# AmandineBtto/NeRAF

Hardware: AMD Instinct MI355X
Metric: field-samples/sec (rays + RIR STFT bins) (higher is better)
Workload: dtype f16; 1 GPU; RAF FurnishedRoom joint training step (BASELINE configs[2]): 4096 rays + 2048 RIR slices x 513 bins per GPU; radiance + grid refresh + ResNet3D + NAcF + STFT loss, backward, GradScaler + fused Adam...; rays_per_gpu=4096, slices_per_gpu=2048, global_rays=4096, global_slices=2048, parallelism=dp1, distinct_resident_batches=16, deterministic=True

## Files before the change

include/neraf_hip.h:

```cpp
#ifndef NERAF_HIP_H
#define NERAF_HIP_H

#include <stddef.h>
#include <stdint.h>

#ifdef __cplusplus
extern "C" {
#endif

typedef struct neraf_ctx neraf_ctx;
typedef void* neraf_stream_t;

enum {
  NERAF_OK = 0,
  NERAF_EINVAL = -1,
  NERAF_EHIP = -2,
  NERAF_ENOGPU = -3,
  NERAF_ESTATE = -4
};

#define NERAF_ABI_VERSION 1

int neraf_abi_version(void);
int neraf_ctx_create(neraf_ctx** out, int device);
void neraf_ctx_destroy(neraf_ctx* ctx);
const char* neraf_last_error(neraf_ctx* ctx);

int neraf_graph_stats(neraf_ctx* ctx, int* captures, int* launches);
int neraf_prof_enable(neraf_ctx* ctx, int on);
int neraf_prof_summary(neraf_ctx* ctx, int kernel_id, double* total_ms, int* launches, double* work);
int neraf_prof_summary_ex(neraf_ctx* ctx, int kernel_id, double* total_ms, int* launches, double* work, double* exec_work);
int neraf_prof_event_overhead(neraf_ctx* ctx, void* scratch_word, neraf_stream_t stream, double* ms);
const char* neraf_prof_kernel_name(int kernel_id);

int neraf_gemm_f16(neraf_ctx* ctx, const void* A, int lda, const void* B, int ldb, int M, int N, int K,
                   int Mpad, int Npad, float alpha, const float* bias, int act,
                   void* C16, int ldc16, void* C16T, int ldc16t, float* C32, int ldc32,
                   neraf_stream_t stream);

int neraf_gemm_f16_grouped(neraf_ctx* ctx, int ngroups, const void* const* A, const void* const* B, const int* M, const int* N,
                           float* const* C32, const int* ldc32, int lda, int ldb, int K, float alpha, const float* alpha_dev,
                           int c32_beta, void* splitk_ws, size_t splitk_bytes, neraf_stream_t stream);

int neraf_gemm_bf16(neraf_ctx* ctx, const void* A, int lda, const void* B, int ldb, int M, int N, int K,
                    int Mpad, int Npad, float alpha, const float* bias, int act,
                    void* C16, int ldc16, void* C16T, int ldc16t, float* C32, int ldc32,
                    neraf_stream_t stream);
int neraf_gemm_bf16_tn(neraf_ctx* ctx, const void* A, const void* B, int M, int N, int K, float* C32, void* splitk_ws,
                       size_t splitk_bytes, neraf_stream_t stream);

typedef struct neraf_nacf_desc {
  int n_feat;
  int n_query;
  int W;
  int C;
  int F;
  int dense_l0;
} neraf_nacf_desc;

size_t neraf_nacf_packed_bytes(const neraf_nacf_desc* d);
size_t neraf_nacf_workspace_bytes(const neraf_nacf_desc* d, int B, int training);

int neraf_nacf_pack_weights(neraf_ctx* ctx, const neraf_nacf_desc* d, const float* const* weights,
                            void* packed, neraf_stream_t stream);

int neraf_nacf_encode_queries(neraf_ctx* ctx, const neraf_nacf_desc* d, const int64_t* time_query,
                              const double* mic_pose, const double* source_pose, const double* rot,
                              const float* aabb_host, int max_len, int B, void* workspace, int training,
                              neraf_stream_t stream);
int neraf_nacf_encode_queries_ex(neraf_ctx* ctx, const neraf_nacf_desc* d, const int64_t* time_query,
                                 const double* mic_pose, const double* source_pose, const double* rot, int pose_rows,
                                 const float* aabb_host, int max_len, int B, void* workspace, int training,
                                 neraf_stream_t stream);

int neraf_nacf_fwd(neraf_ctx* ctx, const neraf_nacf_desc* d, const void* packed, const float* const* weights,
                   const float* feat, int B, float* out, void* workspace, int training, neraf_stream_t stream);

int neraf_nacf_fwd_dense(neraf_ctx* ctx, const neraf_nacf_desc* d, const void* packed, const float* h, int B,
                         float* out, void* workspace, int training, neraf_stream_t stream);

int neraf_nacf_bwd(neraf_ctx* ctx, const neraf_nacf_desc* d, const void* packed, const float* const* weights,
                   const float* feat, int B, const float* out, const float* dout, float* const* grads,
                   float* dfeat, void* workspace, neraf_stream_t stream);

int neraf_nacf_bwd_dense(neraf_ctx* ctx, const neraf_nacf_desc* d, const void* packed, int B, const float* out,
                         const float* dout, float* const* grads, float* dh, void* workspace,
                         neraf_stream_t stream);

#define NERAF_STFT_SUMS_FLOATS (4 + 4 * 256)
int neraf_stft_loss_fwd(neraf_ctx* ctx, const float* pred, const float* gt, size_t n, int loss_type,
                        float* sums, float* losses, neraf_stream_t stream);
int neraf_stft_loss_sums(neraf_ctx* ctx, const float* pred, const float* gt, size_t n, int loss_type,
                         float* sums, neraf_stream_t stream);
int neraf_stft_loss_finalize(neraf_ctx* ctx, const float* sums, size_t n_total, const float* weights, float* losses,
                             neraf_stream_t stream);
// ... 200 lines not shown
```

neraf_amd/_lib.py:

```python
from __future__ import annotations

import ctypes as C
import os
from typing import Dict, Optional

_HERE = os.path.dirname(os.path.abspath(__file__))
LIB_PATH = os.environ.get("NERAF_HIP_LIB") or os.path.join(_HERE, "libneraf_hip.so")

_lib: Optional[C.CDLL] = None
_ctxs: Dict[int, C.c_void_p] = {}

c_fpp = C.POINTER(C.c_void_p)


class GridDesc(C.Structure):
    _fields_ = [("n_levels", C.c_int), ("base_res", C.c_int), ("max_res", C.c_int), ("log2_hashmap_size", C.c_int),
                ("n_features", C.c_int)]


class ResnetDesc(C.Structure):
    _fields_ = [("grid_size", C.c_int), ("in_channels", C.c_int), ("n_features", C.c_int)]


class NacfDesc(C.Structure):
    _fields_ = [("n_feat", C.c_int), ("n_query", C.c_int), ("W", C.c_int), ("C", C.c_int), ("F", C.c_int),
                ("dense_l0", C.c_int)]


SIGNATURES = {
    "neraf_abi_version": (C.c_int, []),
    "neraf_ctx_create": (C.c_int, [C.POINTER(C.c_void_p), C.c_int]),
    "neraf_ctx_destroy": (None, [C.c_void_p]),
    "neraf_last_error": (C.c_char_p, [C.c_void_p]),
    "neraf_gemm_f16": (C.c_int, [C.c_void_p, C.c_void_p, C.c_int, C.c_void_p, C.c_int, C.c_int, C.c_int, C.c_int,
                                 C.c_int, C.c_int, C.c_float, C.c_void_p, C.c_int, C.c_void_p, C.c_int, C.c_void_p,
                                 C.c_int, C.c_void_p, C.c_int, C.c_void_p]),
    "neraf_gemm_f16_grouped": (C.c_int, [C.c_void_p, C.c_int, c_fpp, c_fpp, C.POINTER(C.c_int), C.POINTER(C.c_int), c_fpp,
                                         C.POINTER(C.c_int), C.c_int, C.c_int, C.c_int, C.c_float, C.c_void_p, C.c_int, C.c_void_p, C.c_size_t,
                                         C.c_void_p]),
    "neraf_gemm_bf16": (C.c_int, [C.c_void_p, C.c_void_p, C.c_int, C.c_void_p, C.c_int, C.c_int, C.c_int, C.c_int,
                                  C.c_int, C.c_int, C.c_float, C.c_void_p, C.c_int, C.c_void_p, C.c_int, C.c_void_p,
                                  C.c_int, C.c_void_p, C.c_int, C.c_void_p]),
    "neraf_gemm_bf16_tn": (C.c_int, [C.c_void_p, C.c_void_p, C.c_void_p, C.c_int, C.c_int, C.c_int, C.c_void_p, C.c_void_p, C.c_size_t,
                                     C.c_void_p]),
    "neraf_fused_adam_chunk": (C.c_int, []),
    "neraf_grads_nonfinite": (C.c_int, [C.c_void_p, C.c_void_p, C.c_void_p, C.c_void_p, C.c_void_p, C.c_int, C.c_void_p, C.c_void_p, C.c_int,
                                        C.c_int, C.c_void_p]),
    "neraf_fused_adam": (C.c_int, [C.c_void_p, C.c_void_p, C.c_void_p, C.c_void_p, C.c_void_p, C.c_int, C.c_void_p, C.c_int, C.c_int,
                                   C.c_double, C.c_double, C.c_double, C.c_void_p, C.c_void_p, C.c_void_p, C.c_void_p]),
    "neraf_fused_adam_dual": (C.c_int, [C.c_void_p, C.c_void_p, C.c_void_p, C.c_void_p, C.c_void_p, C.c_int, C.c_void_p, C.c_int, C.c_int,
                                        C.c_double, C.c_double, C.c_double, C.c_void_p, C.c_void_p, C.c_void_p, C.c_void_p, C.c_void_p,
                                        C.c_void_p, C.c_void_p, C.c_int, C.c_void_p, C.c_int, C.c_void_p]),
    "neraf_nacf_packed_bytes": (C.c_size_t, [C.POINTER(NacfDesc)]),
    "neraf_nacf_workspace_bytes": (C.c_size_t, [C.POINTER(NacfDesc), C.c_int, C.c_int]),
    "neraf_nacf_pack_weights": (C.c_int, [C.c_void_p, C.POINTER(NacfDesc), c_fpp, C.c_void_p, C.c_void_p]),
    "neraf_nacf_encode_queries": (C.c_int, [C.c_void_p, C.POINTER(NacfDesc), C.c_void_p, C.c_void_p, C.c_void_p,
                                            C.c_void_p, C.POINTER(C.c_float), C.c_int, C.c_int, C.c_void_p, C.c_int,
                                            C.c_void_p]),
    "neraf_nacf_encode_queries_ex": (C.c_int, [C.c_void_p, C.POINTER(NacfDesc), C.c_void_p, C.c_void_p, C.c_void_p,
                                               C.c_void_p, C.c_int, C.POINTER(C.c_float), C.c_int, C.c_int, C.c_void_p, C.c_int,
                                               C.c_void_p]),
    "neraf_nacf_fwd": (C.c_int, [C.c_void_p, C.POINTER(NacfDesc), C.c_void_p, c_fpp, C.c_void_p, C.c_int, C.c_void_p,
                                 C.c_void_p, C.c_int, C.c_void_p]),
    "neraf_nacf_fwd_dense": (C.c_int, [C.c_void_p, C.POINTER(NacfDesc), C.c_void_p, C.c_void_p, C.c_int, C.c_void_p,
                                       C.c_void_p, C.c_int, C.c_void_p]),
    "neraf_nacf_bwd": (C.c_int, [C.c_void_p, C.POINTER(NacfDesc), C.c_void_p, c_fpp, C.c_void_p, C.c_int, C.c_void_p,
                                 C.c_void_p, c_fpp, C.c_void_p, C.c_void_p, C.c_void_p]),
    "neraf_nacf_bwd_dense": (C.c_int, [C.c_void_p, C.POINTER(NacfDesc), C.c_void_p, C.c_int, C.c_void_p, C.c_void_p,
                                       c_fpp, C.c_void_p, C.c_void_p, C.c_void_p]),
    "neraf_stft_loss_fwd": (C.c_int, [C.c_void_p, C.c_void_p, C.c_void_p, C.c_size_t, C.c_int, C.c_void_p, C.c_void_p,
                                      C.c_void_p]),
    "neraf_stft_loss_sums": (C.c_int, [C.c_void_p, C.c_void_p, C.c_void_p, C.c_size_t, C.c_int, C.c_void_p, C.c_void_p]),
    "neraf_stft_loss_finalize": (C.c_int, [C.c_void_p, C.c_void_p, C.c_size_t, C.c_void_p, C.c_void_p, C.c_void_p]),
    "neraf_stft_loss_bwd": (C.c_int, [C.c_void_p, C.c_void_p, C.c_void_p, C.c_size_t, C.c_size_t, C.c_int, C.c_void_p,
                                      C.c_void_p, C.c_void_p, C.c_void_p, C.c_float, C.c_void_p, C.c_void_p]),
    "neraf_prof_event_overhead": (C.c_int, [C.c_void_p, C.c_void_p, C.c_void_p, C.POINTER(C.c_double)]),
    "neraf_graph_stats": (C.c_int, [C.c_void_p, C.POINTER(C.c_int), C.POINTER(C.c_int)]),
    "neraf_prof_enable": (C.c_int, [C.c_void_p, C.c_int]),
    "neraf_prof_summary": (C.c_int, [C.c_void_p, C.c_int, C.POINTER(C.c_double), C.POINTER(C.c_int), C.POINTER(C.c_double)]),
    "neraf_prof_summary_ex": (C.c_int, [C.c_void_p, C.c_int, C.POINTER(C.c_double), C.POINTER(C.c_int), C.POINTER(C.c_double),
                                        C.POINTER(C.c_double)]),
    "neraf_prof_kernel_name": (C.c_char_p, [C.c_int]),
    "neraf_grid_layout": (C.c_int, [C.POINTER(GridDesc), C.POINTER(C.c_float), C.POINTER(C.c_int), C.POINTER(C.c_uint32),
                                    C.POINTER(C.c_uint32)]),
    "neraf_hash_encode": (C.c_int, [C.c_void_p, C.POINTER(GridDesc), C.c_void_p, C.c_void_p, C.c_longlong, C.c_void_p, C.c_void_p]),
    "neraf_sample_uniform": (C.c_int, [C.c_void_p, C.c_int, C.c_int, C.c_float, C.c_float, C.c_void_p, C.c_uint64, C.c_void_p,
                                       C.c_void_p, C.c_void_p]),
    "neraf_proposal_density": (C.c_int, [C.c_void_p, C.POINTER(GridDesc), C.c_void_p, C.c_void_p, C.c_void_p, C.c_void_p,
                                         C.c_void_p, C.c_int, C.c_int, C.c_float, C.c_int, C.c_void_p, C.c_void_p]),
    "neraf_proposal_density_ex": (C.c_int, [C.c_void_p, C.POINTER(GridDesc), C.c_void_p, C.c_void_p, C.c_void_p, C.c_void_p,
                                            C.c_void_p, C.c_int64, C.c_int, C.c_int, C.c_float, C.c_int, C.c_void_p, C.c_void_p]),
    "neraf_pdf_resample_ex": (C.c_int, [C.c_void_p, C.c_void_p, C.c_void_p, C.c_void_p, C.c_int64, C.c_int, C.c_int, C.c_float,
# ... 163 lines not shown
```

neraf_amd/csrc/common.h:

```cpp
#pragma once
#include <hip/hip_runtime.h>
#include <stdint.h>
#include <stdio.h>
#include <new>
#include <string>
#include <vector>

#include "../../include/neraf_hip.h"

typedef _Float16 half_t;
typedef _Float16 half8 __attribute__((ext_vector_type(8)));
typedef _Float16 half4 __attribute__((ext_vector_type(4)));
typedef _Float16 half2v __attribute__((ext_vector_type(2)));
typedef __bf16 bf16_t;
typedef __bf16 bf16x8 __attribute__((ext_vector_type(8)));
typedef __bf16 bf16x4 __attribute__((ext_vector_type(4)));
typedef float f32x4 __attribute__((ext_vector_type(4)));
typedef float f32x16 __attribute__((ext_vector_type(16)));

enum { PROF_GEMM128 = 0, PROF_GEMM64 = 1, PROF_PROP_DENSITY = 2, PROF_FIELD_QUERY = 3, PROF_CONV = 4, PROF_PROP_BWD = 5, PROF_FIELD_BWD = 6,
       PROF_FIELD_SCATTER = 7, PROF_GEMM_WIDE = 8, PROF_WGRAD = 9, PROF_GEMM64_BF16 = 10, PROF_GEMM12864 = 11,
       PROF_CONV64_BF16 = 12, PROF_CONV12864 = 13, PROF_CONV128 = 14, PROF_CONV_STEM = 15, PROF_NUM_KERNELS = 16 };

struct ProfRec { hipEvent_t a, b; int kid; double work; double exec; };
// ... 123 lines not shown
  if (!words) return;
  size_t blocks = (words + 256 - 1) / 256;
  if (blocks > 4096) blocks = 4096;
  hipLaunchKernelGGL(neraf_zero3_kernel, dim3((unsigned)blocks), dim3(256), 0, st, (unsigned*)p0, w0, (unsigned*)p1, w1, (unsigned*)p2, w2);
}

static inline bool neraf_deterministic() {
  static const bool d = [] { const char* e = getenv("NERAF_DETERMINISTIC"); return e && atoi(e) != 0; }();
  return d;
}

static inline int round_up(int x, int m) { return (x + m - 1) / m * m; }
static inline size_t round_up_sz(size_t x, size_t m) { return (x + m - 1) / m * m; }

enum { ACT_NONE = 0, ACT_LEAKY = 1, ACT_TANH10 = 2, ACT_RELU = 3 };

struct ConvGeom {
  int loader;
  int din, dout, stride, pad, ksize, cin;
  int tflip;
  int tstride;
  int tclass;
  const half_t* zero_page;
};

struct GemmParams {
  const half_t* A; int lda;
  const half_t* B; int ldb;
  int M, N, K;
  int Mpad, Npad;
  float alpha;
  const float* alpha_dev;
  const float* bias;
  int act;
  const half_t* lmask; int ldmask;
  float mask_slope;
  const half_t* add16; int ldadd;
  half_t* C16; int ldc16;
  half_t* C16T; int ldc16t;
  float* C32; int ldc32;
  int c32_beta;
  float* colsum;
  float* colsumsq;
  int stat_rep, stat_stride;
  int stat_det;
  const half_t* bnb_x; int ldbnb;
  const half_t* bnb_mask;
  const float* bnb_fin; int bnb_cpad;
  ConvGeom conv;
  float* splitk_ws; size_t splitk_ws_bytes;
  int tile_n;
  double alg_flops;
  int bf16;
  int ngroups;
  struct Group { const half_t* A; const half_t* B; float* C32; int M, N, ldc32; int tile_begin; } grp[6];
};
constexpr int kMaxGemmGroups = 6;

int launch_gemm_f16(neraf_ctx* ctx, const GemmParams& p, hipStream_t stream);

struct WgradItem {
  const void* dy;
  const void* x;
  float* out;
  int cout, cin, cin_real, ksize, stride, pad, din, dout;
  int K;
  int alpha_idx;
};
int launch_wgrad_grouped(neraf_ctx* ctx, const WgradItem* items, int n, const half_t* zero_page, float* slab_ws, size_t slab_bytes,
                         const float* alpha_dev, hipStream_t stream, bool bf16 = false);

constexpr int kAmaxRep = 32, kAmaxStride = 64;
```

neraf_amd/csrc/gemm_f16.hip:

```cpp
#include "common.h"
#include <stdlib.h>
#include <type_traits>

namespace {

constexpr int BK = 64;

__device__ __forceinline__ float act_apply(float v, int act) {
  if (act == ACT_LEAKY) return v > 0.f ? v : 0.1f * v;
  if (act == ACT_TANH10) return 10.f * tanhf(v);
  if (act == ACT_RELU) return v > 0.f ? v : 0.f;
  return v;
}

template <bool BF> struct ET;
template <> struct ET<false> {
  typedef _Float16 s; typedef half8 v8; typedef half4 v4;
  static __device__ __forceinline__ f32x4 mfma(v8 a, v8 b, f32x4 c) { return __builtin_amdgcn_mfma_f32_16x16x32_f16(a, b, c, 0, 0, 0); }
};
template <> struct ET<true> {
  typedef __bf16 s; typedef bf16x8 v8; typedef bf16x4 v4;
  static __device__ __forceinline__ f32x4 mfma(v8 a, v8 b, f32x4 c) { return __builtin_amdgcn_mfma_f32_16x16x32_bf16(a, b, c, 0, 0, 0); }
};

// ... 679 lines not shown
  __shared__ float tile2[32][33];
  if (p.bnb_x) {
#pragma unroll
    for (int r = 0; r < 4; ++r) tile2[row][c4 + r] = v[r] * (((float)xv[r] - mu[r]) * rsqrtf(var[r] + 1e-5f));
  }
  if (p.C16) {
    E4 h;
#pragma unroll
    for (int r = 0; r < 4; ++r) h[r] = (E)v[r];
    *reinterpret_cast<E4*>(reinterpret_cast<E*>(p.C16) + (size_t)m * p.ldc16 + n) = h;
  }
  if (C32 && m < M) {
    float* dst = C32 + (size_t)m * ldc32 + n;
    if (n + 3 < N && (reinterpret_cast<size_t>(dst) & 15) == 0) {
      f32x4 o = v;
      if (p.c32_beta) o += *reinterpret_cast<const f32x4*>(dst);
      *reinterpret_cast<f32x4*>(dst) = o;
    } else {
#pragma unroll
      for (int r = 0; r < 4; ++r) if (n + r < N) dst[r] = v[r] + (p.c32_beta ? dst[r] : 0.f);
    }
  }
  __syncthreads();
  const int tx = t & 31, ty = t >> 5;
  if (p.C16T) {
#pragma unroll
    for (int i = 0; i < 4; ++i) {
      const int nn = n0 + ty + i * 8, mm = m0 + tx;
      reinterpret_cast<E*>(p.C16T)[(size_t)nn * p.ldc16t + mm] = (E)tile[tx][ty + i * 8];
    }
  }
  if ((p.colsum || p.colsumsq) && ty < 2) {
    float cs = 0.f;
    if (ty == 0) {
#pragma unroll 8
      for (int i = 0; i < 32; ++i) cs += tile[i][tx];
    } else if (p.bnb_x) {
#pragma unroll 8
      for (int i = 0; i < 32; ++i) cs += tile2[i][tx];
    } else {
#pragma unroll 8
      for (int i = 0; i < 32; ++i) { const float x = tile[i][tx]; cs += x * x; }
    }
    float* dst = ty == 0 ? p.colsum : p.colsumsq;
    if (p.stat_det) {
      if (dst) dst[(size_t)blockIdx.y * p.stat_stride + n0 + tx] = cs;
    } else {
      const int rep = p.stat_rep > 1 ? (blockIdx.y & (p.stat_rep - 1)) * p.stat_stride : 0;
      if (dst) atomicAdd(dst + rep + n0 + tx, cs);
    }
  }
}

static void gemm_manifest(neraf_ctx* ctx, const GemmParams& p, int loader, int splits, int bm, int bn, double flops, bool wide = false) {
  double out_elems = (double)p.M * p.N;
  double rA = loader == 0 ? (double)p.M * p.K * 2.0 : (double)p.conv.din * p.conv.din * p.conv.din * p.conv.cin * 2.0;
  double rB = (double)p.N * p.K * 2.0;
  const int ng = p.ngroups > 1 ? p.ngroups : 1;
  if (ng > 1) {
    out_elems = rA = rB = 0.0;
    for (int g = 0; g < ng; ++g) { out_elems += (double)p.grp[g].M * p.grp[g].N; rA += (double)p.grp[g].M * p.K * 2.0; rB += (double)p.grp[g].N * p.K * 2.0; }
  }
  const double epi_r = out_elems * 2.0 * ((p.add16 ? 1 : 0) + (p.lmask ? 1 : 0) + (p.bnb_mask ? 1 : 0) + (p.bnb_x ? 1 : 0));
  const double epi_w = out_elems * (2.0 * ((p.C16 ? 1 : 0) + (p.C16T ? 1 : 0)) + (p.C32 ? 4.0 : 0.0));
  const double slabs = (double)splits * ng * p.Mpad * p.Npad * 4.0;
  char nm[96];
  if (ng > 1)
    snprintf(nm, sizeof(nm), "gemm_f16_nt_pipe_kernel<%d, %d | plain, %d groups, %.0f results K=%d%s", bm, bn, ng, out_elems, p.K, splits > 1 ? " splitK" : "");
  else
    snprintf(nm, sizeof(nm), "%s<%d, %d | %s M=%d N=%d K=%d%s", wide ? "gemm_f16_nt_wide_kernel" : "gemm_f16_nt_pipe_kernel", bm, bn,
             loader == 0 ? "plain" : (p.conv.tflip ? "dgrad" : "conv"), p.M, p.N, p.K, splits > 1 ? " splitK" : "");
  if (splits > 1) {
    neraf_node(ctx, nm, flops, rA + rB, slabs);
    neraf_node(ctx, "splitk_reduce_kernel | K-split slabs -> result", 0.0, slabs + epi_r, epi_w);
  } else {
    neraf_node(ctx, nm, flops, rA + rB + epi_r, epi_w);
  }
}

template <int BM, int BN, int NST, int LOADER, int KS, bool BF, bool TC = false, int NW = 4, bool GRP = false>
int launch_pipe(neraf_ctx* ctx, const GemmParams& p_in, int splits, hipStream_t stream) {
  using PT = PipeTile<BM, BN, NST>;
  GemmParams p = p_in;
  if ((p.ngroups > 1) != GRP) return neraf_fail(ctx, NERAF_EINVAL, "gemm: grouped launches take the grouped instantiation");
  int grp_tiles = 0;
  if (GRP) {
    for (int g = 0; g < p.ngroups; ++g) {
      p.grp[g].tile_begin = grp_tiles;
      grp_tiles += ((p.grp[g].M + BM - 1) / BM) * ((p.grp[g].N + BN - 1) / BN);
    }
  }
  static bool attr_set = false;
  if (!attr_set) {
    NERAF_HIP_CHECK(ctx, hipFuncSetAttribute(reinterpret_cast<const void*>(&gemm_f16_nt_pipe_kernel<BM, BN, NST, LOADER, KS, BF, TC, NW, GRP>),
                                             hipFuncAttributeMaxDynamicSharedMemorySize, PT::LDS_BYTES));
    attr_set = true;
  }
  const int ng = p.ngroups > 1 ? p.ngroups : 1;
  const int ntiles = GRP ? grp_tiles : (p.Mpad / BM) * (p.Npad / BN);
  double flops = 2.0 * p.M * p.N * p.K;
  if (ng > 1) { flops = 0.0; for (int g = 0; g < ng; ++g) flops += 2.0 * p.grp[g].M * p.grp[g].N * p.K; }
  const double exec_flops = (LOADER != 0 && p.conv.tstride > 1) ? (p.alg_flops > 0.0 ? p.alg_flops : flops) : flops;
  if (p.alg_flops > 0.0) flops = p.alg_flops;
  constexpr int kid = LOADER == 2 ? PROF_CONV_STEM
                      : LOADER == 1 ? (BM * BN == 128 * 128 ? PROF_CONV128 : (BM == 128 ? PROF_CONV12864 : (BF ? PROF_CONV64_BF16 : PROF_CONV)))
                                    : (BM * BN == 128 * 128 ? PROF_GEMM128 : (BM == 128 ? PROF_GEMM12864 : (BF ? PROF_GEMM64_BF16 : PROF_GEMM64)));
  ProfScope prof(ctx, stream, kid, flops, exec_flops);
  hipLaunchKernelGGL((gemm_f16_nt_pipe_kernel<BM, BN, NST, LOADER, KS, BF, TC, NW, GRP>), dim3(ntiles * splits), dim3(NW * 64), PT::LDS_BYTES,
                     stream, p, splits);
  NERAF_HIP_CHECK(ctx, hipGetLastError());
  if (ctx && ctx->manifest) gemm_manifest(ctx, p, LOADER, splits, BM, BN, flops);
  if (splits > 1) {
    hipLaunchKernelGGL(splitk_reduce_kernel<BF>, dim3(p.Npad / 32, p.Mpad / 32, ng), dim3(256), 0, stream, p, splits);
    NERAF_HIP_CHECK(ctx, hipGetLastError());
  }
  return NERAF_OK;
}


template <int BM, int BN, int NST, bool BF>
int launch_wide(neraf_ctx* ctx, const GemmParams& p, int splits, hipStream_t stream) {
  using T = Tile<BM, BN, 4>;
  constexpr int LDS_BYTES = (NST * T::STAGE_BYTES > T::NWAVES * T::EPI_BYTES_WAVE) ? NST * T::STAGE_BYTES : T::NWAVES * T::EPI_BYTES_WAVE;
  static_assert(LDS_BYTES <= 160 * 1024, "LDS budget");
  static bool attr_set = false;
  if (!attr_set) {
    NERAF_HIP_CHECK(ctx, hipFuncSetAttribute(reinterpret_cast<const void*>(&gemm_f16_nt_wide_kernel<BM, BN, NST, BF>),
                                             hipFuncAttributeMaxDynamicSharedMemorySize, LDS_BYTES));
    attr_set = true;
  }
  const int ntiles = (p.Mpad / BM) * (p.Npad / BN);
  ProfScope prof(ctx, stream, PROF_GEMM_WIDE, p.alg_flops > 0.0 ? p.alg_flops : 2.0 * p.M * p.N * p.K, 2.0 * p.M * p.N * p.K);
  hipLaunchKernelGGL((gemm_f16_nt_wide_kernel<BM, BN, NST, BF>), dim3(ntiles * splits), dim3(512), LDS_BYTES, stream, p, splits);
  NERAF_HIP_CHECK(ctx, hipGetLastError());
  if (ctx && ctx->manifest) gemm_manifest(ctx, p, 0, splits, BM, BN, p.alg_flops > 0.0 ? p.alg_flops : 2.0 * p.M * p.N * p.K, true);
  if (splits > 1) {
    hipLaunchKernelGGL(splitk_reduce_kernel<BF>, dim3(p.Npad / 32, p.Mpad / 32, 1), dim3(256), 0, stream, p, splits);
    NERAF_HIP_CHECK(ctx, hipGetLastError());
  }
  return NERAF_OK;
}

struct WgDesc {
  const void* dy; const void* x; float* out;
  unsigned long long slab_off;
  int block_begin; int K;
  unsigned short cout, cin, cin_real, taps, din, tiles_n, splits;
  unsigned char dl, stride, ksize, loader; signed char pad; unsigned char mh, ai, r2, r3, r4;
};
static_assert(sizeof(WgDesc) == 64, "descriptor table must fit the 4 KiB kernel-argument segment");
constexpr int kMaxWg = 56;
struct WgTable { int n; int total_blocks; const half_t* zero_page; const float* alpha_dev; float* slab; int order; WgDesc d[kMaxWg]; };

__device__ __forceinline__ int wg_find(const WgTable& t, int bid) {
  int lo = 0, hi = t.n - 1;
  while (lo < hi) { const int mid = (lo + hi + 1) >> 1; if (t.d[mid].block_begin <= bid) lo = mid; else hi = mid - 1; }
  return lo;
}

__device__ __forceinline__ size_t wg_out_index(const WgDesc& d, int m, int n) {
  const int tap = n / d.cin, c = n - tap * d.cin;
  return ((size_t)m * d.cin_real + c) * d.taps + tap;
}

template <bool BF> struct TrRead;
template <> struct TrRead<true> {
  static __device__ __forceinline__ bf16x4 rd(const char* p) {
    return __builtin_amdgcn_ds_read_tr16_b64_v4bf16((__attribute__((address_space(3))) bf16x4*)p);
  }
};
template <> struct TrRead<false> {
  typedef __fp16 fp16x4 __attribute__((ext_vector_type(4)));
  static __device__ __forceinline__ half4 rd(const char* p) {
    const fp16x4 v = __builtin_amdgcn_ds_read_tr16_b64_v4f16((__attribute__((address_space(3))) fp16x4*)p);
    return __builtin_bit_cast(half4, v);
  }
};

template <int NST, bool BF>
__global__ __launch_bounds__(256) void wgrad_grouped_tn_kernel(WgTable t) {
  using E = typename ET<BF>::s; using E4 = typename ET<BF>::v4; using E8 = typename ET<BF>::v8;
  constexpr int BM = 64, BN = 64;
  constexpr int STAGE_BYTES = (BM + BN) * 128;
  extern __shared__ __attribute__((aligned(16))) char smem[];
  const int tid = threadIdx.x;
  const int lane = tid & 63;
  const int wave = __builtin_amdgcn_readfirstlane(tid >> 6);
  const int wm = wave >> 1, wn = wave & 1;
  const int gi = wg_find(t, blockIdx.x);
  const WgDesc& D = t.d[gi];
  int bid = blockIdx.x - D.block_begin;
  const int splits = D.splits, tiles_n = D.tiles_n, tiles_m = D.cout / BM;
  const int split = bid % splits;
// ... 366 lines not shown
    const f32x4 v = *reinterpret_cast<const f32x4*>(im + row * IM_LD + col);
    *reinterpret_cast<f32x4*>(slab + (size_t)(m_base + row) * Npad + n_base + col) = v;
  }
}

struct WgRedTable { int n; const float* alpha_dev; const float* slab; int tile_begin[kMaxWg + 1]; unsigned char item[kMaxWg]; };

__device__ __forceinline__ int wg_red_cb(const WgDesc& D) { return D.taps == 1 ? (D.cin < 256 ? D.cin : 256) : (D.taps > 32 ? D.cin : (D.cin < 128 ? D.cin : 128)); }

__global__ __launch_bounds__(256) void wgrad_grouped_reduce_kernel(WgTable t, WgRedTable r) {
  __shared__ float blk[3584];
  int lo = 0, hi = r.n - 1;
  const int bid = blockIdx.x;
  while (lo < hi) { const int mid = (lo + hi + 1) >> 1; if (r.tile_begin[mid] <= bid) lo = mid; else hi = mid - 1; }
  const WgDesc& D = t.d[r.item[lo]];
  const int tile = bid - r.tile_begin[lo];
  const int taps = D.taps, cin = D.cin, CB = wg_red_cb(D), cbs = cin / CB;
  const int m = tile / cbs, ci0 = (tile - m * cbs) * CB;
  const int Npad = D.tiles_n * 64;
  const size_t slab = (size_t)D.cout * Npad;
  const float* src = r.slab + D.slab_off + (size_t)m * Npad + ci0;
  const int splits = D.splits, pitch = taps + 1, q4 = CB >> 2, total4 = q4 * taps;
  for (int e = threadIdx.x; e < total4; e += 256) {
    const int tap = e / q4, c = (e - tap * q4) * 4;
    const float* p = src + tap * cin + c;
    f32x4 v = f32x4{0.f, 0.f, 0.f, 0.f};
    int s2 = 0;
    for (; s2 + 8 <= splits; s2 += 8) {
      f32x4 a[8];
#pragma unroll
      for (int u = 0; u < 8; ++u) a[u] = *reinterpret_cast<const f32x4*>(p + (size_t)(s2 + u) * slab);
#pragma unroll
      for (int u = 0; u < 8; ++u) v += a[u];
    }
    for (; s2 < splits; ++s2) v += *reinterpret_cast<const f32x4*>(p + (size_t)s2 * slab);
#pragma unroll
    for (int k = 0; k < 4; ++k) blk[taps == 1 ? c + k : (c + k) * pitch + tap] = v[k];
  }
  __syncthreads();
  const float alpha = r.alpha_dev ? r.alpha_dev[D.ai] : 1.f;
  const int creal = (D.cin_real - ci0) < CB ? (D.cin_real - ci0) : CB;
  float* dst = D.out + ((size_t)m * D.cin_real + ci0) * taps;
  for (int j = threadIdx.x; j < creal * taps; j += 256) {
    const int c = j / taps, tap = j - c * taps;
    dst[j] = blk[taps == 1 ? c : c * pitch + tap] * alpha;
  }
}

static const int kWide = [] { const char* e = getenv("NERAF_GEMM_WIDE"); return e ? atoi(e) : 1; }();
static const int kSplitMinK = [] { const char* e = getenv("NERAF_SPLIT_MIN_K"); return e ? atoi(e) : 32; }();

static bool conv_waves8() { static const bool v = [] { const char* e = getenv("NERAF_CONV_WAVES"); return e && atoi(e) == 8; }(); return v; }

template <int LOADER, int KS, bool BF>
int dispatch_tile(neraf_ctx* ctx, const GemmParams& p_in, hipStream_t stream) {
  GemmParams p = p_in;
  const int cus = ctx ? ctx->num_cus : 256;
  static const int kTclass = [] { const char* e = getenv("NERAF_DGRAD_TCLASS"); return e ? atoi(e) : 1; }();
  p.conv.tclass = 0;
  if (LOADER == 1 && kTclass && p.conv.tstride == 2 && p.conv.tflip && (p.conv.dout & 1) == 0 && p.ngroups <= 1 &&
      p.Mpad == p.conv.dout * p.conv.dout * p.conv.dout && (p.Mpad % 512) == 0 && (p.Npad % 64) == 0 && !p.lmask && !p.C16T && !p.C32 &&
      !p.colsum && !p.colsumsq) {
    p.conv.tclass = 1;
    if constexpr (LOADER == 1) { if (conv_waves8()) return launch_pipe<64, 64, 4, LOADER, KS, BF, true, 8>(ctx, p, 1, stream); }
    return launch_pipe<64, 64, 4, LOADER, KS, BF, LOADER == 1>(ctx, p, 1, stream);
  }
  const int nk = p.K / BK;
  int bm = 128, bn = 128;
  const bool can128 = (p.Mpad % 128) == 0 && (p.Npad % 128) == 0;
  static const int kTile64 = [] { const char* e = getenv("NERAF_CONV_TILE64"); return e ? atoi(e) : 1; }();
  if (p.tile_n == 64 && (p.Mpad % 128) == 0 && !(kTile64 && LOADER == 1)) { bm = 128; bn = 64; }
  else if (!can128 || (p.Mpad / 128) * (p.Npad / 128) < cus) { bm = 64; bn = 64; }
  const int ng = p.ngroups > 1 ? p.ngroups : 1;
  int ntiles = (p.Mpad / bm) * (p.Npad / bn);
  bool uniform = true;
  if (ng > 1) {
    bm = 64; bn = 64; ntiles = 0;
    for (int g = 0; g < ng; ++g) {
      ntiles += (round_up(p.grp[g].M, 64) / 64) * (round_up(p.grp[g].N, 64) / 64);
      uniform = uniform && round_up(p.grp[g].M, 64) == p.Mpad && round_up(p.grp[g].N, 64) == p.Npad;
    }
  }
  int splits = 1;
  static const int kOversub = [] { const char* e = getenv("NERAF_SPLIT_OVERSUB"); const int v = e ? atoi(e) : 2; return v < 1 ? 1 : (v > 4 ? 4 : v); }();
  if (p.splitk_ws && uniform && ntiles * 2 <= cus && nk >= kSplitMinK) {
    splits = ((LOADER != 0 && ntiles >= 64) ? kOversub : 1) * cus / ntiles;
    if (splits > nk / 4) splits = nk / 4;
    if (splits > 128) splits = 128;
    while (splits >= 2 && (size_t)splits * ng * p.Mpad * p.Npad * 4 > p.splitk_ws_bytes) splits >>= 1;
    if (splits < 2) splits = 1;
  }
  if (LOADER == 0 && ng == 1 && kWide && (p.Mpad % 256) == 0) {
    if ((p.Npad % 160) == 0 && (p.Mpad / 256) * (p.Npad / 160) * 4 >= cus * 3) return launch_wide<256, 160, 3, BF>(ctx, p, 1, stream);
    if ((p.Npad % 128) == 0 && (p.Mpad / 256) * (p.Npad / 128) >= cus) return launch_wide<256, 128, 3, BF>(ctx, p, 1, stream);
  }
  if (LOADER == 0 && ng == 1 && kWide && bm == 128 && bn == 128 && splits == 1 && ntiles < 2 * cus)
    return launch_wide<128, 128, 3, BF>(ctx, p, 1, stream);
  static const int kTile32 = [] { const char* e = getenv("NERAF_TILE32"); return e ? atoi(e) : 128; }();
  if constexpr (LOADER == 0) {
    if (ng > 1) {
      if (kTile32 && splits == 1 && ntiles <= kTile32) return launch_pipe<32, 32, 4, LOADER, KS, BF, false, 4, true>(ctx, p, 1, stream);
      return launch_pipe<64, 64, 4, LOADER, KS, BF, false, 4, true>(ctx, p, splits, stream);
    }
    if (kTile32 && splits == 1 && bm == 64 && bn == 64 && ntiles <= kTile32 && !p.C16T)
      return launch_pipe<32, 32, 4, LOADER, KS, BF>(ctx, p, 1, stream);
  }
  if (bm == 128 && bn == 128) return launch_pipe<128, 128, 2, LOADER, KS, BF>(ctx, p, splits, stream);
  if (bm == 128 && bn == 64) return launch_pipe<128, 64, 3, LOADER, KS, BF>(ctx, p, splits, stream);
  if constexpr (LOADER == 1) { if (conv_waves8()) return launch_pipe<64, 64, 4, LOADER, KS, BF, false, 8>(ctx, p, splits, stream); }
  return launch_pipe<64, 64, 4, LOADER, KS, BF>(ctx, p, splits, stream);
}

}

int launch_wgrad_grouped(neraf_ctx* ctx, const WgradItem* items, int n, const half_t* zero_page, float* slab_ws, size_t slab_bytes,
                         const float* alpha_dev, hipStream_t stream, bool bf16) {
  if (n <= 0 || n > kMaxWg || !items || !zero_page) return neraf_fail(ctx, NERAF_EINVAL, "wgrad_grouped: bad arguments");
  static const int nst = [] { const char* e = getenv("NERAF_WGRAD_NST"); const int v = e ? atoi(e) : 3; return v < 2 ? 2 : (v > 4 ? 4 : v); }();
// ... 120 lines not shown
    if ((p.Mpad && p.Mpad != round_up(p.grp[0].M, 64)) || (p.Npad && p.Npad != round_up(p.grp[0].N, 64)))
      return neraf_fail(ctx, NERAF_EINVAL, "gemm: a grouped launch's Mpad / Npad, if given, are group 0's M / N rounded up to 64");
    p.A = p.grp[0].A; p.B = p.grp[0].B; p.C32 = p.grp[0].C32; p.ldc32 = p.grp[0].ldc32;
    p.M = p.grp[0].M; p.N = p.grp[0].N; p.Mpad = round_up(p.M, 64); p.Npad = round_up(p.N, 64);
  }
  if ((p.Mpad % 64) != 0 || (p.Npad % 64) != 0 || p.M > p.Mpad || p.N > p.Npad || p.M <= 0 || p.N <= 0)
    return neraf_fail(ctx, NERAF_EINVAL, "gemm: Mpad/Npad must be multiples of 64 covering M/N");
  if (!p.stat_det && p.stat_rep > 1 && (p.stat_rep & (p.stat_rep - 1))) return neraf_fail(ctx, NERAF_EINVAL, "gemm: stat_rep must be a power of two");
  if ((p.conv.loader == 0 && (p.lda % 8)) || (p.ldb % 8) || (p.C16 && (p.ldc16 % 8)) || (p.C16T && (p.ldc16t % 8)) ||
      (p.lmask && (p.ldmask % 4)))
    return neraf_fail(ctx, NERAF_EINVAL, "gemm: leading dimensions must keep 16-byte alignment");
  switch (p.conv.loader) {
    case 0: return p.bf16 ? dispatch_tile<0, 1, true>(ctx, p, stream) : dispatch_tile<0, 1, false>(ctx, p, stream);
    case 1:
      if ((p.conv.cin % 64) || !p.conv.zero_page) return neraf_fail(ctx, NERAF_EINVAL, "conv loader 1: cin % 64 and zero page");
      if (p.conv.ksize == 3) return p.bf16 ? dispatch_tile<1, 3, true>(ctx, p, stream) : dispatch_tile<1, 3, false>(ctx, p, stream);
      if (p.conv.ksize == 1) return p.bf16 ? dispatch_tile<1, 1, true>(ctx, p, stream) : dispatch_tile<1, 1, false>(ctx, p, stream);
      return neraf_fail(ctx, NERAF_EINVAL, "conv loader 1: ksize must be 1 or 3");
    case 2:
      if (p.conv.cin != 8 || p.conv.ksize != 5 || !p.conv.zero_page || p.bf16) return neraf_fail(ctx, NERAF_EINVAL, "conv loader 2: cin 8, ksize 5, fp16");
      return dispatch_tile<2, 5, false>(ctx, p, stream);
  }
  return neraf_fail(ctx, NERAF_EINVAL, "gemm: unknown loader");
}

extern "C" int neraf_gemm_f16(neraf_ctx* ctx, const void* A, int lda, const void* B, int ldb, int M, int N, int K,
                              int Mpad, int Npad, float alpha, const float* bias, int act, void* C16, int ldc16,
                              void* C16T, int ldc16t, float* C32, int ldc32, neraf_stream_t stream) {
  GemmParams p{};
  p.A = (const half_t*)A; p.lda = lda; p.B = (const half_t*)B; p.ldb = ldb;
  p.M = M; p.N = N; p.K = K; p.Mpad = Mpad; p.Npad = Npad; p.alpha = alpha; p.bias = bias; p.act = act;
  p.C16 = (half_t*)C16; p.ldc16 = ldc16; p.C16T = (half_t*)C16T; p.ldc16t = ldc16t; p.C32 = C32; p.ldc32 = ldc32;
  return launch_gemm_f16(ctx, p, (hipStream_t)stream);
}

extern "C" int neraf_gemm_f16_grouped(neraf_ctx* ctx, int ngroups, const void* const* A, const void* const* B, const int* M, const int* N,
                                      float* const* C32, const int* ldc32, int lda, int ldb, int K, float alpha, const float* alpha_dev,
                                      int c32_beta, void* splitk_ws, size_t splitk_bytes, neraf_stream_t stream) {
  if (ngroups < 1 || ngroups > kMaxGemmGroups || !A || !B || !M || !N || !C32 || !ldc32)
    return neraf_fail(ctx, NERAF_EINVAL, "gemm_f16_grouped: 1 to 6 groups");
  GemmParams p{};
  p.lda = lda; p.ldb = ldb; p.K = K; p.alpha = alpha; p.alpha_dev = alpha_dev; p.c32_beta = c32_beta;
  p.splitk_ws = (float*)splitk_ws; p.splitk_ws_bytes = splitk_ws ? splitk_bytes : 0;
  for (int g = 0; g < ngroups; ++g) {
    if (M[g] <= 0 || N[g] <= 0) return neraf_fail(ctx, NERAF_EINVAL, "gemm_f16_grouped: M and N must be positive");
    GemmParams::Group& G = p.grp[g];
    G.A = (const half_t*)A[g]; G.B = (const half_t*)B[g]; G.C32 = C32[g]; G.M = M[g]; G.N = N[g]; G.ldc32 = ldc32[g];
    if (!G.A || !G.B || !G.C32) return neraf_fail(ctx, NERAF_EINVAL, "gemm_f16_grouped: null operand or result");
  }
  p.ngroups = ngroups;
  return launch_gemm_f16(ctx, p, (hipStream_t)stream);
}

extern "C" int neraf_gemm_bf16(neraf_ctx* ctx, const void* A, int lda, const void* B, int ldb, int M, int N, int K,
                               int Mpad, int Npad, float alpha, const float* bias, int act, void* C16, int ldc16,
                               void* C16T, int ldc16t, float* C32, int ldc32, neraf_stream_t stream) {
  GemmParams p{};
  p.bf16 = 1;
  p.A = (const half_t*)A; p.lda = lda; p.B = (const half_t*)B; p.ldb = ldb;
  p.M = M; p.N = N; p.K = K; p.Mpad = Mpad; p.Npad = Npad; p.alpha = alpha; p.bias = bias; p.act = act;
  p.C16 = (half_t*)C16; p.ldc16 = ldc16; p.C16T = (half_t*)C16T; p.ldc16t = ldc16t; p.C32 = C32; p.ldc32 = ldc32;
  return launch_gemm_f16(ctx, p, (hipStream_t)stream);
}

extern "C" int neraf_gemm_bf16_tn(neraf_ctx* ctx, const void* A, const void* B, int M, int N, int K, float* C32, void* splitk_ws,
                                  size_t splitk_bytes, neraf_stream_t stream) {
  if (!A || !B || !C32 || M <= 0 || N <= 0 || K <= 0 || (M % 64) || (N % 64) || (K % 64) || !splitk_ws || splitk_bytes < 256)
    return neraf_fail(ctx, NERAF_EINVAL, "gemm_bf16_tn: M, N, K multiples of 64; scratch required");
  WgradItem it{};
  it.dy = A; it.x = B; it.out = C32;
  it.cout = M; it.cin = N; it.cin_real = N; it.ksize = 1; it.stride = 1; it.pad = 0; it.din = 1; it.dout = 1; it.K = K;
  return launch_wgrad_grouped(ctx, &it, 1, (const half_t*)splitk_ws, (float*)((char*)splitk_ws + 256), splitk_bytes - 256, nullptr,
                              (hipStream_t)stream, true);
}
```

Measured before the change: 263.6 million field-samples/s.

## Add persistent streaming GEMM body for tall-skinny f16 GEMMs with LDS-resident weights

```diff
diff --git a/include/neraf_hip.h b/include/neraf_hip.h
--- a/include/neraf_hip.h
+++ b/include/neraf_hip.h
@@ -41,6 +41,11 @@
 int neraf_gemm_f16_grouped(neraf_ctx* ctx, int ngroups, const void* const* A, const void* const* B, const int* M, const int* N,
                            float* const* C32, const int* ldc32, int lda, int ldb, int K, float alpha, const float* alpha_dev,
                            int c32_beta, void* splitk_ws, size_t splitk_bytes, neraf_stream_t stream);
+
+int neraf_gemm_f16_stream(neraf_ctx* ctx, const void* A, int lda, const void* B, int ldb, int M, int N, int K, int Mpad, int Npad,
+                          float alpha, const float* bias, const void* add16, int ldadd, void* C16, int ldc16, void* C16T,
+                          int ldc16t, float* C32, int ldc32, float* colsum, float* colsumsq, int stat_rep, int stat_stride,
+                          int stat_det, int body, int max_workgroups, neraf_stream_t stream);
 
 int neraf_gemm_bf16(neraf_ctx* ctx, const void* A, int lda, const void* B, int ldb, int M, int N, int K,
                     int Mpad, int Npad, float alpha, const float* bias, int act,
diff --git a/neraf_amd/_lib.py b/neraf_amd/_lib.py
--- a/neraf_amd/_lib.py
+++ b/neraf_amd/_lib.py
@@ -38,6 +38,9 @@
     "neraf_gemm_f16_grouped": (C.c_int, [C.c_void_p, C.c_int, c_fpp, c_fpp, C.POINTER(C.c_int), C.POINTER(C.c_int), c_fpp,
                                          C.POINTER(C.c_int), C.c_int, C.c_int, C.c_int, C.c_float, C.c_void_p, C.c_int, C.c_void_p, C.c_size_t,
                                          C.c_void_p]),
+    "neraf_gemm_f16_stream": (C.c_int, [C.c_void_p, C.c_void_p, C.c_int, C.c_void_p, C.c_int, C.c_int, C.c_int, C.c_int, C.c_int, C.c_int,
+                                        C.c_float, C.c_void_p, C.c_void_p, C.c_int, C.c_void_p, C.c_int, C.c_void_p, C.c_int, C.c_void_p,
+                                        C.c_int, C.c_void_p, C.c_void_p, C.c_int, C.c_int, C.c_int, C.c_int, C.c_int, C.c_void_p]),
     "neraf_gemm_bf16": (C.c_int, [C.c_void_p, C.c_void_p, C.c_int, C.c_void_p, C.c_int, C.c_int, C.c_int, C.c_int,
                                   C.c_int, C.c_int, C.c_float, C.c_void_p, C.c_int, C.c_void_p, C.c_int, C.c_void_p,
                                   C.c_int, C.c_void_p, C.c_int, C.c_void_p]),
diff --git a/neraf_amd/csrc/common.h b/neraf_amd/csrc/common.h
--- a/neraf_amd/csrc/common.h
+++ b/neraf_amd/csrc/common.h
@@ -199,6 +199,7 @@
   int tile_n;
   double alg_flops;
   int bf16;
+  int stream_body, stream_max_wg;
   int ngroups;
   struct Group { const half_t* A; const half_t* B; float* C32; int M, N, ldc32; int tile_begin; } grp[6];
 };
diff --git a/neraf_amd/csrc/gemm_f16.hip b/neraf_amd/csrc/gemm_f16.hip
--- a/neraf_amd/csrc/gemm_f16.hip
+++ b/neraf_amd/csrc/gemm_f16.hip
@@ -755,7 +755,7 @@
   }
 }
 
-static void gemm_manifest(neraf_ctx* ctx, const GemmParams& p, int loader, int splits, int bm, int bn, double flops, bool wide = false) {
+static void gemm_manifest(neraf_ctx* ctx, const GemmParams& p, int loader, int splits, int bm, int bn, double flops, bool wide = false, bool stream = false) {
   double out_elems = (double)p.M * p.N;
   double rA = loader == 0 ? (double)p.M * p.K * 2.0 : (double)p.conv.din * p.conv.din * p.conv.din * p.conv.cin * 2.0;
   double rB = (double)p.N * p.K * 2.0;
@@ -771,7 +771,8 @@
   if (ng > 1)
     snprintf(nm, sizeof(nm), "gemm_f16_nt_pipe_kernel<%d, %d | plain, %d groups, %.0f results K=%d%s", bm, bn, ng, out_elems, p.K, splits > 1 ? " splitK" : "");
   else
-    snprintf(nm, sizeof(nm), "%s<%d, %d | %s M=%d N=%d K=%d%s", wide ? "gemm_f16_nt_wide_kernel" : "gemm_f16_nt_pipe_kernel", bm, bn,
+    snprintf(nm, sizeof(nm), "%s<%d, %d | %s M=%d N=%d K=%d%s",
+             stream ? "gemm_f16_nt_stream_kernel" : (wide ? "gemm_f16_nt_wide_kernel" : "gemm_f16_nt_pipe_kernel"), bm, bn,
              loader == 0 ? "plain" : (p.conv.tflip ? "dgrad" : "conv"), p.M, p.N, p.K, splits > 1 ? " splitK" : "");
   if (splits > 1) {
     neraf_node(ctx, nm, flops, rA + rB, slabs);
@@ -842,6 +843,196 @@
     NERAF_HIP_CHECK(ctx, hipGetLastError());
   }
   return NERAF_OK;
+}
+
+constexpr int kStreamRows = 64;
+constexpr int stream_slices(int n) { return n > 128 ? n / 128 : 1; }
+
+__device__ __forceinline__ float row16_sum(float x) {
+  x += __builtin_bit_cast(float, __builtin_amdgcn_mov_dpp(__builtin_bit_cast(int, x), 0xB1, 0xF, 0xF, true));
+  x += __builtin_bit_cast(float, __builtin_amdgcn_mov_dpp(__builtin_bit_cast(int, x), 0x4E, 0xF, 0xF, true));
+  x += __builtin_bit_cast(float, __builtin_amdgcn_mov_dpp(__builtin_bit_cast(int, x), 0x141, 0xF, 0xF, true));
+  x += __builtin_bit_cast(float, __builtin_amdgcn_mov_dpp(__builtin_bit_cast(int, x), 0x140, 0xF, 0xF, true));
+  return x;
+}
+
+template <int N, int K, bool STATS>
+__global__ __launch_bounds__(512) void gemm_f16_nt_stream_kernel(GemmParams p, int nblocks, int nrg) {
+  constexpr int R = kStreamRows, KB = K / 32;
+  constexpr int CS = stream_slices(N), NW = N / CS, FNW = NW / 16;
+  constexpr int CPRB = K / 8, SWZ = (CPRB - 1) & 15;
+  constexpr int BCH = NW * CPRB / 512;
+  constexpr int IC = 64, NPASS = NW / IC, FNP = IC / 16, IMG_LD = IC + 8, CPR = IC / 8, IMG_WAVE = 16 * IMG_LD * 2;
+  static_assert(N * K <= 16384 && N % 64 == 0 && K % 64 == 0 && NW <= 128 && BCH >= 1, "B must fit 32 KiB of LDS");
+  static_assert(8 * 2 * NW * 4 <= 8 * IMG_WAVE, "the statistics' reduction re-uses the result images");
+  __shared__ __attribute__((aligned(16))) char bs[NW * K * 2];
+  __shared__ __attribute__((aligned(16))) char img_all[8 * IMG_WAVE];
+
+  const int tid = threadIdx.x;
+  const int lane = tid & 63;
+  const int wave = __builtin_amdgcn_readfirstlane(tid >> 6);
+  const int g = wave >> 2, w4 = wave & 3;
+  const int frow = lane & 15, fq = lane >> 4;
+  int rg, cs;
+  if (CS > 1 && (nrg & 7) == 0) { const int q = blockIdx.x >> 3; cs = q % CS; rg = (q / CS) * 8 + (blockIdx.x & 7); }
+  else { rg = blockIdx.x / CS; cs = blockIdx.x - rg * CS; }
+  const int n_w0 = cs * NW;
+  const int nv = 2 * nrg;
+
+  auto load_a = [&](int blk, half8 (&xa)[KB]) {
+    const half_t* src = p.A + (size_t)(blk * R + w4 * 16 + frow) * p.lda + fq * 8;
+#pragma unroll
+    for (int kb = 0; kb < KB; ++kb) xa[kb] = *reinterpret_cast<const half8*>(src + kb * 32);
+  };
+
+  int b = 2 * rg + g;
+  half8 xa[KB], xn[KB];
+  {
+    uint4 bv[BCH];
+#pragma unroll
+    for (int i = 0; i < BCH; ++i) {
+      const int c = i * 512 + tid, row = c / CPRB, ch = c % CPRB;
+      bv[i] = *reinterpret_cast<const uint4*>(p.B + (size_t)(n_w0 + row) * p.ldb + ch * 8);
+    }
+    if (b < nblocks) load_a(b, xa);
+#pragma unroll
+    for (int i = 0; i < BCH; ++i) {
+      const int c = i * 512 + tid, row = c / CPRB, ch = c % CPRB;
+      *reinterpret_cast<uint4*>(bs + row * (K * 2) + ((ch ^ (row & SWZ)) * 16)) = bv[i];
+    }
+  }
+  __syncthreads();
+
+  const float alpha = p.alpha;
+  half_t* im = reinterpret_cast<half_t*>(img_all + wave * IMG_WAVE);
+  const char* b_lane = bs + frow * (K * 2);
+  f32x4 s[STATS ? FNW : 1], s2[STATS ? FNW : 1];
+#pragma unroll
+  for (int j = 0; j < (STATS ? FNW : 1); ++j) s[j] = s2[j] = f32x4{0.f, 0.f, 0.f, 0.f};
+
+  for (; b < nblocks; b += nv) {
+    const int bnext = b + nv;
+    if (bnext < nblocks) load_a(bnext, xn);
+
+    f32x4 acc[FNW];
+#pragma unroll
+    for (int j = 0; j < FNW; ++j) acc[j] = f32x4{0.f, 0.f, 0.f, 0.f};
+#pragma unroll
+    for (int kb = 0; kb < KB; ++kb) {
+      const int coff = ((kb * 4 + fq) ^ (frow & SWZ)) * 16;
+#pragma unroll
+      for (int j = 0; j < FNW; ++j) {
+        const half8 wb = *reinterpret_cast<const half8*>(b_lane + j * 16 * (K * 2) + coff);
+        acc[j] = __builtin_amdgcn_mfma_f32_16x16x32_f16(wb, xa[kb], acc[j], 0, 0, 0);
+      }
+    }
+
+    const int row0 = b * R + w4 * 16;
+    const int m = row0 + frow;
+    const bool live = m < p.M;
+#pragma unroll
+    for (int pass = 0; pass < NPASS; ++pass) {
+      half4 ad[FNP];
+      if (p.add16) {
+#pragma unroll
+        for (int j = 0; j < FNP; ++j)
+          ad[j] = *reinterpret_cast<const half4*>(p.add16 + (size_t)m * p.ldadd + n_w0 + pass * IC + j * 16 + fq * 4);
+      }
+#pragma unroll
+      for (int j = 0; j < FNP; ++j) {
+        const int jj = pass * FNP + j;
+        f32x4 v = acc[jj] * alpha;
+        if (p.add16) {
+#pragma unroll
+          for (int r = 0; r < 4; ++r) v[r] += (float)ad[j][r];
+        }
+#pragma unroll
+        for (int r = 0; r < 4; ++r) if (!live) v[r] = 0.f;
+        if constexpr (STATS) { s[jj] += v; s2[jj] += v * v; }
+        half4 h;
+#pragma unroll
+        for (int r = 0; r < 4; ++r) h[r] = (half_t)v[r];
+        *reinterpret_cast<half4*>(im + frow * IMG_LD + j * 16 + fq * 4) = h;
+      }
+      asm volatile("s_waitcnt lgkmcnt(0)" ::: "memory");
+#pragma unroll
+      for (int it = 0; it < 16 * CPR / 64; ++it) {
+        const int idx = it * 64 + lane, row = idx / CPR, ch = idx - row * CPR;
+        const uint4 d = *reinterpret_cast<const uint4*>(im + row * IMG_LD + ch * 8);
+        *reinterpret_cast<uint4*>(p.C16 + (size_t)(row0 + row) * p.ldc16 + n_w0 + pass * IC + ch * 8) = d;
+      }
+      asm volatile("s_waitcnt lgkmcnt(0)" ::: "memory");
+    }
+    if (bnext < nblocks) {
+#pragma unroll
+      for (int kb = 0; kb < KB; ++kb) xa[kb] = xn[kb];
+    }
+  }
+
+  if constexpr (STATS) {
+    __syncthreads();
+    float* red = reinterpret_cast<float*>(img_all);
+#pragma unroll
+    for (int j = 0; j < FNW; ++j)
+#pragma unroll
+      for (int r = 0; r < 4; ++r) {
+        const float x = row16_sum(s[j][r]), y = row16_sum(s2[j][r]);
+        if (frow == 0) {
+          const int col = j * 16 + fq * 4 + r;
+          red[(wave * 2 + 0) * NW + col] = x;
+          red[(wave * 2 + 1) * NW + col] = y;
+        }
+      }
+    __syncthreads();
+    if (tid < 2 * NW) {
+      const int which = tid / NW, col = tid - which * NW;
+      float v = 0.f;
+#pragma unroll
+      for (int w = 0; w < 8; ++w) v += red[(w * 2 + which) * NW + col];
+      float* dst = which ? p.colsumsq : p.colsum;
+      if (dst) {
+        if (p.stat_det) dst[(size_t)((2 * rg * R) >> 5) * p.stat_stride + n_w0 + col] = v;
+        else atomicAdd(dst + (p.stat_rep > 1 ? (rg & (p.stat_rep - 1)) * p.stat_stride : 0) + n_w0 + col, v);
+      }
+    }
+  }
+}
+
+static bool stream_qualifies(const GemmParams& p) {
+  const bool nk = (p.N == 64 || p.N == 128 || p.N == 256) && (p.K == 64 || p.K == 128 || p.K == 256) && p.N * p.K <= 16384;
+  return nk && p.Npad == p.N && p.conv.loader == 0 && p.ngroups <= 1 && !p.bf16 && (p.Mpad % kStreamRows) == 0 && p.C16 &&
+         !p.bias && !p.act && !p.lmask && !p.C16T && !p.C32 && !p.alpha_dev && !p.bnb_x && !p.bnb_mask &&
+         (!p.add16 || (p.ldadd % 4) == 0);
+}
+
+template <int N, int K>
+int launch_stream_nk(neraf_ctx* ctx, const GemmParams& p, hipStream_t stream) {
+  const int nblocks = p.Mpad / kStreamRows;
+  constexpr int CS = stream_slices(N);
+  int nrg = (ctx ? ctx->num_cus : 256) / CS;
+  if (p.stream_max_wg > 0 && nrg > p.stream_max_wg / CS) nrg = p.stream_max_wg / CS;
+  if (nrg > (nblocks + 1) / 2) nrg = (nblocks + 1) / 2;
+  if (nrg < 1) nrg = 1;
+  const int grid = nrg * CS;
+  const double flops = p.alg_flops > 0.0 ? p.alg_flops : 2.0 * p.M * p.N * p.K;
+  ProfScope prof(ctx, stream, N == 64 ? PROF_GEMM12864 : PROF_GEMM_WIDE, flops, 2.0 * p.M * p.N * p.K);
+  if (p.colsum || p.colsumsq) hipLaunchKernelGGL((gemm_f16_nt_stream_kernel<N, K, true>), dim3(grid), dim3(512), 0, stream, p, nblocks, nrg);
+  else hipLaunchKernelGGL((gemm_f16_nt_stream_kernel<N, K, false>), dim3(grid), dim3(512), 0, stream, p, nblocks, nrg);
+  NERAF_HIP_CHECK(ctx, hipGetLastError());
+  if (ctx && ctx->manifest) gemm_manifest(ctx, p, 0, 1, N, K, flops, false, true);
+  return NERAF_OK;
+}
+
+int launch_stream(neraf_ctx* ctx, const GemmParams& p, hipStream_t stream) {
+  switch (p.N * 1000 + p.K) {
+    case 64064: return launch_stream_nk<64, 64>(ctx, p, stream);
+    case 64128: return launch_stream_nk<64, 128>(ctx, p, stream);
+    case 64256: return launch_stream_nk<64, 256>(ctx, p, stream);
+    case 128064: return launch_stream_nk<128, 64>(ctx, p, stream);
+    case 128128: return launch_stream_nk<128, 128>(ctx, p, stream);
+    case 256064: return launch_stream_nk<256, 64>(ctx, p, stream);
+  }
+  return neraf_fail(ctx, NERAF_EINVAL, "gemm: shape outside the streaming body's");
 }
 
 struct WgDesc {
@@ -1314,6 +1505,8 @@
 
 static bool conv_waves8() { static const bool v = [] { const char* e = getenv("NERAF_CONV_WAVES"); return e && atoi(e) == 8; }(); return v; }
 
+constexpr int kStreamMinM = 32768;
+
 template <int LOADER, int KS, bool BF>
 int dispatch_tile(neraf_ctx* ctx, const GemmParams& p_in, hipStream_t stream) {
   GemmParams p = p_in;
@@ -1326,6 +1519,13 @@
     p.conv.tclass = 1;
     if constexpr (LOADER == 1) { if (conv_waves8()) return launch_pipe<64, 64, 4, LOADER, KS, BF, true, 8>(ctx, p, 1, stream); }
     return launch_pipe<64, 64, 4, LOADER, KS, BF, LOADER == 1>(ctx, p, 1, stream);
+  }
+  if (p.stream_body == 1 && !(LOADER == 0 && !BF && stream_qualifies(p)))
+    return neraf_fail(ctx, NERAF_EINVAL, "gemm: shape or epilogue outside the streaming body's");
+  if constexpr (LOADER == 0 && !BF) {
+    const bool det_stats = p.stat_det && (p.colsum || p.colsumsq);
+    if (p.stream_body != 2 && stream_qualifies(p) && (p.stream_body == 1 || (p.Mpad >= kStreamMinM && !det_stats)))
+      return launch_stream(ctx, p, stream);
   }
   const int nk = p.K / BK;
   int bm = 128, bn = 128;
@@ -1552,6 +1752,22 @@
   return launch_gemm_f16(ctx, p, (hipStream_t)stream);
 }
 
+extern "C" int neraf_gemm_f16_stream(neraf_ctx* ctx, const void* A, int lda, const void* B, int ldb, int M, int N, int K, int Mpad, int Npad,
+                                     float alpha, const float* bias, const void* add16, int ldadd, void* C16, int ldc16, void* C16T,
+                                     int ldc16t, float* C32, int ldc32, float* colsum, float* colsumsq, int stat_rep, int stat_stride,
+                                     int stat_det, int body, int max_workgroups, neraf_stream_t stream) {
+  if (body < 0 || body > 2 || max_workgroups < 0) return neraf_fail(ctx, NERAF_EINVAL, "gemm_f16_stream: body 0..2, max_workgroups >= 0");
+  GemmParams p{};
+  p.A = (const half_t*)A; p.lda = lda; p.B = (const half_t*)B; p.ldb = ldb;
+  p.M = M; p.N = N; p.K = K; p.Mpad = Mpad; p.Npad = Npad; p.alpha = alpha; p.bias = bias;
+  p.add16 = (const half_t*)add16; p.ldadd = ldadd;
+  p.C16 = (half_t*)C16; p.ldc16 = ldc16; p.C16T = (half_t*)C16T; p.ldc16t = ldc16t; p.C32 = C32; p.ldc32 = ldc32;
+  p.colsum = colsum; p.colsumsq = colsumsq; p.stat_rep = stat_rep; p.stat_stride = stat_stride; p.stat_det = stat_det;
+  p.tile_n = N == 64 ? 64 : 0;
+  p.stream_body = body; p.stream_max_wg = max_workgroups;
+  return launch_gemm_f16(ctx, p, (hipStream_t)stream);
+}
+
 extern "C" int neraf_gemm_bf16(neraf_ctx* ctx, const void* A, int lda, const void* B, int ldb, int M, int N, int K,
                                int Mpad, int Npad, float alpha, const float* bias, int act, void* C16, int ldc16,
                                void* C16T, int ldc16t, float* C32, int ldc32, neraf_stream_t stream) {
```

New measurement: 269.9 million field-samples/s (median of 6 runs). 2.4% higher.
